# mahfuzalhasan/WaveFormer

Measured on AMD Instinct MI355X. Metric: 128³×4 volumes/sec fwd (1/2/4/8 MI355X) + Dice Δ vs reference, higher is better.
Workload: dtype bf16x3; 1 GPU; MultiscaleTransformer (WaveFormer encoder) forward, 128^3x4 crops; global_batch=8, per_gpu_batch=8, precision=bf16x3, parallelism=replicas x1 (no data-path collective), hip_graph=True

## Files before the change

### waveformer_amd/csrc/ffn.hip

```cpp
#include "kernels.hpp"

namespace wf {

template <typename T>
struct Store4;
template <>
struct Store4<uint16_t> {
  typedef bf16x4 vec;
  static __device__ __forceinline__ f32x4 up(vec u) {
    return f32x4{bf2f((uint16_t)u[0]), bf2f((uint16_t)u[1]), bf2f((uint16_t)u[2]),
                 bf2f((uint16_t)u[3])};
  }
  static __device__ __forceinline__ uint16_t down(float v) { return f2bf(v); }
  static __device__ __forceinline__ vec zero() { return vec{0, 0, 0, 0}; }
  static __device__ __forceinline__ void store4(uint16_t* p, f32x4 v) {
    bf16x4 o;
    o[0] = (short)f2bf(v.x);
    o[1] = (short)f2bf(v.y);
    o[2] = (short)f2bf(v.z);
    o[3] = (short)f2bf(v.w);
    *reinterpret_cast<bf16x4*>(p) = o;
  }
};
template <>
// ... 185 lines not shown
  const int yt = t % nty;
  t /= nty;
  const int zt = t % nzs;
  const int b = t / nzs;
  const int x0 = xt * TX, y0 = yt * TY, z0 = zt * ZS, z1 = min(z0 + ZS, D);
  const int c0 = cc * CH;
  const int tid = threadIdx.x;
  const int cp = tid % (CH / 2), xi = tid / (CH / 2);

  f32x2 w2[27];
#pragma unroll
  for (int k = 0; k < 27; ++k) {
    const int kk = FLIP ? 26 - k : k;
    w2[k] = f32x2{w[(c0 + 2 * cp) * 27 + kk], w[(c0 + 2 * cp + 1) * 27 + kk]};
  }
  const f32x2 bv = bias ? f32x2{bias[c0 + 2 * cp], bias[c0 + 2 * cp + 1]} : f32x2{0.f, 0.f};

  if (LN1) {
    for (int i = tid; i < CH; i += 256) {
      l1w[i] = ln1_w[c0 + i];
      l1b[i] = ln1_b[c0 + i];
    }
    __syncthreads();
  }
  typename V::raw stg[NLD];
  f32x2 st1[LN1 ? NLD : 1];
  bool ok1[LN1 ? NLD : 1];
  const T* src = in + (int64_t)b * D * H * W * Hd + c0;
  auto fetch = [&](int p) {
    const bool pz = p >= 0 && p < D;
    const int pc = min(max(p, 0), D - 1);
#pragma unroll
    for (int j = 0; j < NLD; ++j) {
      const int i = min(j * 256 + tid, PY * PX * NV - 1);
      const int pos = i / NV, v = i - pos * NV;
      const int yy = y0 - 1 + pos / PX, xx = x0 - 1 + pos % PX;
      const bool ok = pz && yy >= 0 && yy < H && xx >= 0 && xx < W;
      const int yc = min(max(yy, 0), H - 1), xc = min(max(xx, 0), W - 1);
      const int64_t gp = ((int64_t)pc * H + yc) * W + xc;
      const typename V::raw u = *reinterpret_cast<const typename V::raw*>(src + gp * Hd + V::N * v);
      stg[j] = ok ? u : V::zero();
      if constexpr (LN1) {
        st1[j] = *reinterpret_cast<const f32x2*>(ln1_stats + ((int64_t)b * D * H * W + gp) * 2);
        ok1[j] = ok;
      }
    }
  };
  auto commit = [&](int buf) {
#pragma unroll
    for (int j = 0; j < NLD; ++j) {
      const int i = j * 256 + tid;
      if (i < PY * PX * NV) {
        if constexpr (LN1) {
          const int v = i % NV;
          const f32x4 lw = *reinterpret_cast<const f32x4*>(l1w + 4 * v);
          const f32x4 lb = *reinterpret_cast<const f32x4*>(l1b + 4 * v);
          const f32x4 y = gelu_erf4((stg[j] - st1[j].x) * st1[j].y * lw + lb);
          stg[j] = ok1[j] ? y : V::zero();
        }
        V::put(pl[buf] + (size_t)i * V::N, stg[j]);
      }
    }
  };

  f32x2 accA[TY], accB[TY], accC[TY];
#pragma unroll
  for (int o = 0; o < TY; ++o) accA[o] = accB[o] = accC[o] = f32x2{0.f, 0.f};
  const int xo = x0 + xi;
  double cs0 = 0.0, cs1 = 0.0, cq0 = 0.0, cq1 = 0.0;
  fetch(z0 - 1);
  commit(0);
  __syncthreads();
  int buf = 0;
  for (int p = z0 - 1; p <= z1; ++p) {
    fetch(p + 1);
    const float* P = pl[buf] + xi * CH + 2 * cp;
#pragma unroll
    for (int r = 0; r < PY; ++r) {
      const f32x2 v0 = *reinterpret_cast<const f32x2*>(P + (r * PX + 0) * CH);
      const f32x2 v1 = *reinterpret_cast<const f32x2*>(P + (r * PX + 1) * CH);
      const f32x2 v2 = *reinterpret_cast<const f32x2*>(P + (r * PX + 2) * CH);
#pragma unroll
      for (int ky = 0; ky < 3; ++ky) {
        const int o = r - ky;
        if (o < 0 || o >= TY) continue;
        const f32x2* w0 = w2 + ky * 3;
        accC[o] = w0[2] * v2 + (w0[1] * v1 + (w0[0] * v0 + accC[o]));
        accB[o] = w0[11] * v2 + (w0[10] * v1 + (w0[9] * v0 + accB[o]));
        accA[o] = w0[20] * v2 + (w0[19] * v1 + (w0[18] * v0 + accA[o]));
      }
    }
    const int zo = p - 1;
    if (zo >= z0) {
      f32x2 r1[TY];
#pragma unroll
      for (int o = 0; o < TY; ++o) r1[o] = Store2<T>::round(accA[o] + bv);
      float mu[TY], m2[TY];
      if (pstats) {
#pragma unroll
        for (int o = 0; o < TY; ++o) mu[o] = group_sum<16>(r1[o].x + r1[o].y) * (1.f / 32.f);
#pragma unroll
        for (int o = 0; o < TY; ++o) {
          const float dx = r1[o].x - mu[o], dy = r1[o].y - mu[o];
          m2[o] = group_sum<16>(dx * dx + dy * dy);
        }
      }
      if (xo < W) {
#pragma unroll
        for (int o = 0; o < TY; ++o) {
          const int yo = y0 + o;
          if (yo < H) {
            const int64_t pos = (((int64_t)b * D + zo) * H + yo) * W + xo;
            Store2<T>::put(out + pos * Hd + c0 + 2 * cp, r1[o]);
            if (cstats) {
              const double a0 = (double)r1[o].x, a1 = (double)r1[o].y;
              cs0 += a0;
              cs1 += a1;
              cq0 += a0 * a0;
              cq1 += a1 * a1;
            }
            if (pstats && cp % (DW_STAT_GROUP / 2) == 0)
              *reinterpret_cast<float2*>(pstats + (pos * (ncc * NG) + cc * NG + cp / (DW_STAT_GROUP / 2)) * 2) =
                  float2{mu[o], m2[o]};
          }
        }
      }
    }
#pragma unroll
    for (int o = 0; o < TY; ++o) {
      accA[o] = accB[o];
      accB[o] = accC[o];
      accC[o] = f32x2{0.f, 0.f};
    }
    commit(buf ^ 1);
    __syncthreads();
    buf ^= 1;
  }
  if (cstats) {
    double* red = reinterpret_cast<double*>(&pl[0][0]);
    double* r = red + (xi * (CH / 2) + cp) * 4;
    r[0] = cs0;
    r[1] = cs1;
    r[2] = cq0;
    r[3] = cq1;
    __syncthreads();
    if (tid < CH * 2) {
      const int pc = tid >> 2, mom = tid & 3;
      double t = 0.0;
#pragma unroll
      for (int xx = 0; xx < TX; ++xx) t += red[(xx * (CH / 2) + pc) * 4 + mom];
      const int c = c0 + 2 * pc + (mom & 1);
      atomicAdd(cstats + ((int64_t)b * Hd + c) * 2 + (mom >> 1), t);
    }
  }
}

int launch_dwconv3d(const void* in, const float* w, const float* b, void* out, float* pstats,
                    int B, int Hd, int D, int H, int W, int prec, hipStream_t s, double* cstats,
                    const float* ln1_stats, const float* ln1_w, const float* ln1_b, int flip) {
  if (Hd % DW_CH != 0) return fail(WF_E_SHAPE, "dwconv3d: hidden width must be a multiple of 32");
  if (flip && (ln1_stats || !store32(prec)))
    return fail(WF_E_SHAPE, "dwconv3d: the mirrored taps are for fp32 data without LN1 staging");
  const bool narrow = W <= 8 && Hd % 64 == 0 && store32(prec) && !flip && !ln1_stats;
  const int dch = narrow ? 64 : DW_CH, dtx = narrow ? 8 : DW_TX;
  const int64_t base = (int64_t)B * (Hd / dch) * cdiv(H, DW_TY) * cdiv(W, dtx);
  int ZS = D;
  const int zmin = narrow ? 4 : 8;
  while (ZS > zmin && base * cdiv(D, ZS) < 2048) ZS = (ZS + 1) / 2;
  const int64_t blocks = base * cdiv(D, ZS);
  if (narrow) {
    hipLaunchKernelGGL((dwconv3d_kernel<float, false, false, 64, 8>), dim3((unsigned)blocks),
                       dim3(256), 0, s, reinterpret_cast<const float*>(in), w, b,
                       reinterpret_cast<float*>(out), pstats, B, Hd, D, H, W, ZS, cstats, nullptr,
                       nullptr, nullptr);
  } else if (ln1_stats) {
    if (!store32(prec) || !ln1_w || !ln1_b)
      return fail(WF_E_SHAPE, "dwconv3d: the LN1 staging needs fp32 h1 and LN1 weights");
    hipLaunchKernelGGL((dwconv3d_kernel<float, true>), dim3((unsigned)blocks), dim3(256), 0, s,
                       reinterpret_cast<const float*>(in), w, b, reinterpret_cast<float*>(out),
                       pstats, B, Hd, D, H, W, ZS, cstats, ln1_stats, ln1_w, ln1_b);
  } else if (store32(prec) && flip)
    hipLaunchKernelGGL((dwconv3d_kernel<float, false, true>), dim3((unsigned)blocks), dim3(256),
                       0, s, reinterpret_cast<const float*>(in), w, b,
                       reinterpret_cast<float*>(out), pstats, B, Hd, D, H, W, ZS, cstats,
                       nullptr, nullptr, nullptr);
  else if (store32(prec))
    hipLaunchKernelGGL((dwconv3d_kernel<float, false>), dim3((unsigned)blocks), dim3(256), 0, s,
                       reinterpret_cast<const float*>(in), w, b, reinterpret_cast<float*>(out),
                       pstats, B, Hd, D, H, W, ZS, cstats, nullptr, nullptr, nullptr);
  else
    hipLaunchKernelGGL((dwconv3d_kernel<uint16_t, false>), dim3((unsigned)blocks), dim3(256), 0,
                       s, reinterpret_cast<const uint16_t*>(in), w, b,
                       reinterpret_cast<uint16_t*>(out), pstats, B, Hd, D, H, W, ZS, cstats,
                       nullptr, nullptr, nullptr);
  return check_launch("dwconv3d");
}

__global__ __launch_bounds__(256) void ln_stats_finalize_kernel(const float* __restrict__ ps,
                                                                int np, int group, float eps,
                                                                float* __restrict__ out,
                                                                int64_t M) {
  const int64_t r = (int64_t)blockIdx.x * 256 + threadIdx.x;
  if (r >= M) return;
  const float2* p = reinterpret_cast<const float2*>(ps) + r * np;
  float mu = 0.f;
  for (int i = 0; i < np; ++i) mu += p[i].x;
  mu *= 1.f / np;
  float m2 = 0.f;
  for (int i = 0; i < np; ++i) {
    const float d = p[i].x - mu;
    m2 += p[i].y + (float)group * d * d;
  }
  *reinterpret_cast<float2*>(out + 2 * r) = float2{mu, rsqrtf(m2 / ((float)np * group) + eps)};
}

int launch_ln_stats_finalize(const float* pstats, int np, int group, float eps, float* out,
                             int64_t M, hipStream_t s) {
  hipLaunchKernelGGL(ln_stats_finalize_kernel, dim3((unsigned)cdiv(M, 256)), dim3(256), 0, s,
                     pstats, np, group, eps, out, M);
  return check_launch("ln_stats_finalize");
}

template <typename T>
static void launch_dw(int tw, dim3 grid, dim3 block, size_t lds, hipStream_t s, const void* in,
                      const float* w, const float* b, const float* ln_w, const float* ln_b,
                      float eps, void* out, int B, int Hd, int D, int H, int W, int R) {
  const T* i = reinterpret_cast<const T*>(in);
  T* o = reinterpret_cast<T*>(out);
  switch (tw) {
    case 2: hipLaunchKernelGGL((dwconv_ln_gelu_kernel<2, T>), grid, block, lds, s, i, w, b, ln_w, ln_b, eps, o, B, Hd, D, H, W, R); break;
    case 4: hipLaunchKernelGGL((dwconv_ln_gelu_kernel<4, T>), grid, block, lds, s, i, w, b, ln_w, ln_b, eps, o, B, Hd, D, H, W, R); break;
    case 8: hipLaunchKernelGGL((dwconv_ln_gelu_kernel<8, T>), grid, block, lds, s, i, w, b, ln_w, ln_b, eps, o, B, Hd, D, H, W, R); break;
    default: hipLaunchKernelGGL((dwconv_ln_gelu_kernel<16, T>), grid, block, lds, s, i, w, b, ln_w, ln_b, eps, o, B, Hd, D, H, W, R); break;
  }
}

int launch_dwconv_ln_gelu(const void* in, const float* w, const float* b, const float* ln_w,
                          const float* ln_b, float eps, void* out, int B, int Hd, int D, int H,
                          int W, int prec, hipStream_t s) {
  if (Hd % 4 != 0) return fail(WF_E_SHAPE, "dwconv: hidden width must be a multiple of 4");
  const int nchunk = Hd / 4;
  if (nchunk > 512) return fail(WF_E_SHAPE, "dwconv: hidden width > 2048 is not supported");
  int R = 256 / nchunk;
  if (R < 1) R = 1;
  if (R > H) R = H;
  int TW = Hd >= 1536 ? 8 : 16;
  while (TW > 2 && (size_t)R * TW * (Hd + 4) * 4 > 64 * 1024) TW >>= 1;
  while (R > 1 && (size_t)R * TW * (Hd + 4) * 4 > 64 * 1024) --R;
  const int threads = (int)cdiv((int64_t)nchunk * R, 64) * 64;
  const int tw_eff = TW > W ? W : TW;
  int tw_t = 16;
  if (tw_eff <= 2) tw_t = 2;
  else if (tw_eff <= 4) tw_t = 4;
  else if (tw_eff <= 8) tw_t = 8;
  const size_t lds = ((size_t)R * tw_t * (Hd + 4) + 2 * (size_t)R * tw_t) * 4;
  const int64_t blocks = (int64_t)B * D * cdiv(H, R) * cdiv(W, tw_t);
  if (store32(prec))
    launch_dw<float>(tw_t, dim3((unsigned)blocks), dim3(threads), lds, s, in, w, b, ln_w, ln_b,
                     eps, out, B, Hd, D, H, W, R);
  else
    launch_dw<uint16_t>(tw_t, dim3((unsigned)blocks), dim3(threads), lds, s, in, w, b, ln_w,
                        ln_b, eps, out, B, Hd, D, H, W, R);
  return check_launch("dwconv_ln_gelu");
}

static DwFcArgs dwfc_args(const void* h1, const float* dw_w, const float* dw_b, const float* ln2_w,
                          const float* ln2_b, float eps2, const uint16_t* fc, const float* fc_b,
                          const float* x, const float* stats, const float* n2_w,
                          const float* n2_b, const float* bscale, float* out, int64_t B, int64_t D,
                          int64_t H, int64_t W) {
  DwFcArgs d{};
  d.h1 = h1;
  d.dw_w = dw_w;
  d.dw_b = dw_b;
  d.ln2_w = ln2_w;
  d.ln2_b = ln2_b;
  d.eps2 = eps2;
  d.fc = fc;
  d.fc_b = fc_b;
  d.x = x;
  d.stats = stats;
  d.n2_w = n2_w;
  d.n2_b = n2_b;
  d.bscale = bscale;
  d.out = out;
  d.B = (int)B;
  d.D = (int)D;
  d.H = (int)H;
  d.W = (int)W;
  return d;
}

}

using namespace wf;

extern "C" int64_t wf_ccf_ffn_workspace_bytes(int64_t B, int64_t C, int64_t hidden, int64_t D,
                                              int64_t H, int64_t W, int precision) {
  const int64_t e = store32(precision) ? 4 : 2;
  const int64_t one = ((B * D * H * W * hidden * e) + 255) & ~(int64_t)255;
  const int64_t st = B * D * H * W * (hidden / DW_STAT_GROUP) * 2 * 4;
  const int64_t s1 = B * D * H * W * 2 * 4;
  const int64_t fcs = C == 192 && hidden == 768 && store32(precision) ? DWFC3_FCS_BYTES : 0;
  return 2 * one + 2 * ((st + 255) & ~(int64_t)255) + ((s1 + 255) & ~(int64_t)255) + fcs;
}

extern "C" int wf_ccf_ffn_stage(int stage, const float* xh, const float* stats,
                                const float* n2_w, const float* n2_b,
                                const uint16_t* pw_bf16x2, const float* pw_b,
                                const float* ln1_w, const float* ln1_b, float eps1,
                                const float* dw_w, const float* dw_b, const float* ln2_w,
                                const float* ln2_b, float eps2, const uint16_t* fc_bf16x2,
                                const float* fc_b, const float* branch_scale, float* out,
                                void* workspace, int64_t B, int64_t C, int64_t hidden,
                                int64_t D, int64_t H, int64_t W, int precision, void* stream) {
  const bool keep = (stage & 16) != 0;
  stage &= ~16;
  WF_REQUIRE(stage >= 0 && stage <= 3, "stage must be 0 (all), 1 (pwconv), 2 (dwconv) or 3 (fc)");
  WF_REQUIRE(B >= 1 && D >= 1 && H >= 1 && W >= 1, "empty volume");
  WF_REQUIRE(C % 8 == 0 && hidden % 8 == 0, "C and hidden must be multiples of 8");
  WF_REQUIRE(valid_prec(precision), "unknown precision");
  WF_REQUIRE_PTR(xh);
  WF_REQUIRE_PTR(pw_bf16x2);
  WF_REQUIRE_PTR(ln1_w);
  WF_REQUIRE_PTR(ln1_b);
  WF_REQUIRE_PTR(dw_w);
  WF_REQUIRE_PTR(dw_b);
  WF_REQUIRE_PTR(ln2_w);
  WF_REQUIRE_PTR(ln2_b);
  WF_REQUIRE_PTR(fc_bf16x2);
  WF_REQUIRE_PTR(out);
  WF_REQUIRE_PTR(workspace);
  if (stats) {
    WF_REQUIRE_PTR(n2_w);
    WF_REQUIRE_PTR(n2_b);
  }
  hipStream_t s = (hipStream_t)stream;
  const int64_t M = B * D * H * W;
  const int64_t e = store32(precision) ? 4 : 2;
  const int64_t one = ((M * hidden * e) + 255) & ~(int64_t)255;
  void* h1 = workspace;
  void* h2 = reinterpret_cast<char*>(workspace) + one;
  const int hbf = !store32(precision);

  GemmArgs g{};
  g.prec = precision;
  g.a_src = xh;
  g.a_bf16 = 0;
  g.a_C = (int)C;
  g.a_nseg = 1;
  g.a_map = MAP_IDENTITY;
  g.a_ln = stats ? LN_GIVEN : LN_NONE;
  g.a_stats = stats;
  g.a_ln_w = n2_w;
  g.a_ln_b = n2_b;
  g.w = pw_bf16x2;
  g.M = M;
  g.N = (int)hidden;
  g.K = (int)C;
  g.epi = EPI_LN_GELU;
  g.bias = pw_b;
  g.e_ln_w = ln1_w;
  g.e_ln_b = ln1_b;
  g.e_eps = eps1;
  g.out = h1;
  g.out_bf16 = hbf;
  g.ldo = hidden;
  int rc = 0;
  const bool split_ln1 = store32(precision) && hidden >= 768 && hidden <= 1536 &&
                         !gemm_lnw_wide_shape(g);
  const bool whole = getenv("WF_FFN_FUSED") != nullptr;
  if (!keep && whole && C == 48 && hidden == 192) {
    if (stage == 1 || stage == 3) return 0;
    DwFcArgs d = dwfc_args(nullptr, dw_w, dw_b, ln2_w, ln2_b, eps2, fc_bf16x2, fc_b, xh, stats, n2_w,
                           n2_b, branch_scale, out, B, D, H, W);
    d.pw = pw_bf16x2;
    d.pw_b = pw_b;
    d.ln1_w = ln1_w;
    d.ln1_b = ln1_b;
    d.eps1 = eps1;
    return launch_ffn_fused(d, precision, s);
  }
  static const bool ln1_pass = getenv("WF_FFN_LN1_FUSE") == nullptr;
  const int64_t stq = ((M * (hidden / DW_STAT_GROUP) * 2 * 4) + 255) & ~(int64_t)255;
  float* pw_pst = reinterpret_cast<float*>(reinterpret_cast<char*>(workspace) + 2 * one + stq);
  float* ln1_st = reinterpret_cast<float*>(reinterpret_cast<char*>(workspace) + 2 * one + 2 * stq);
  int pw_np = 0;
  if (split_ln1 && !keep && !ln1_pass && hidden % DW_STAT_GROUP == 0) {
    GemmArgs g2 = g;
    g2.epi = EPI_STORE;
    const int nt = gemm_kc_pick_nt(g2);
    if (nt > 0 && hidden % (16 * nt) == 0) pw_np = (int)(hidden / (16 * nt));
  }
  if (stage == 0 || stage == 1) {
    if (split_ln1 && pw_np > 0) {
      GemmArgs g2 = g;
      g2.epi = EPI_STORE;
      g2.o_pstats = pw_pst;
      rc = launch_gemm(g2, s, "wf_ccf_ffn_fwd(pwconv)");
      if (!rc)
        rc = launch_ln_stats_finalize(pw_pst, pw_np, (int)(hidden / pw_np), eps1, ln1_st, M, s);
    } else if (split_ln1) {
      GemmArgs g2 = g;
      g2.epi = EPI_STORE;
      rc = launch_gemm(g2, s, "wf_ccf_ffn_fwd(pwconv)");
      if (!rc)
        rc = wf_ln_act_fwd(reinterpret_cast<const float*>(h1), ln1_w, ln1_b, eps1, 1,
                           reinterpret_cast<float*>(h1), M, hidden, stream);
    } else {
      rc = launch_gemm(g, s, "wf_ccf_ffn_fwd(pwconv)");
    }
  }
  if (rc) return rc;
  const bool no_dwfc = getenv("WF_FFN_NO_DWFC") != nullptr;
  const bool dwfc1 = C == 48 && hidden == 192, dwfc2 = C == 96 && hidden == 384;
  const bool dwfc3 = C == 192 && hidden == 768 && store32(precision) && ffn_dwfc3_tb_fits(B, D, H, W);
  if (!keep && !no_dwfc && (dwfc1 || dwfc2 || dwfc3)) {
    if (stage == 1 || stage == 3) return rc;
    DwFcArgs d = dwfc_args(h1, dw_w, dw_b, ln2_w, ln2_b, eps2, fc_bf16x2, fc_b, xh, stats, n2_w,
                           n2_b, branch_scale, out, B, D, H, W);
    if (dwfc3)
      d.fcs = reinterpret_cast<uint16_t*>(
          reinterpret_cast<char*>(workspace) +
          wf_ccf_ffn_workspace_bytes(B, C, hidden, D, H, W, precision) - DWFC3_FCS_BYTES);
    return dwfc1   ? launch_ffn_dwfc_s1(d, precision, s)
           : dwfc2 ? launch_ffn_dwfc2(d, precision, s)
                   : launch_ffn_dwfc3(d, precision, s);
  }
  const bool split_ln = hidden % 32 == 0;
  WF_REQUIRE(!keep || split_ln, "training needs hidden % 32 == 0 (h2 kept pre-LayerNorm)");
  float* pst = reinterpret_cast<float*>(reinterpret_cast<char*>(workspace) + 2 * one);
  if (stage == 0 || stage == 2) {
    if (split_ln && split_ln1 && pw_np > 0)
      rc = launch_dwconv3d(h1, dw_w, dw_b, h2, pst, (int)B, (int)hidden, (int)D, (int)H,
                           (int)W, precision, s, nullptr, ln1_st, ln1_w, ln1_b);
    else if (split_ln)
      rc = launch_dwconv3d(h1, dw_w, dw_b, h2, pst, (int)B, (int)hidden, (int)D, (int)H,
                           (int)W, precision, s);
    else
      rc = launch_dwconv_ln_gelu(h1, dw_w, dw_b, ln2_w, ln2_b, eps2, h2, (int)B, (int)hidden,
                                 (int)D, (int)H, (int)W, precision, s);
  }
  if (rc || stage == 1 || stage == 2) return rc;
  GemmArgs f{};
  f.prec = precision;
  f.a_src = h2;
  f.a_bf16 = hbf;
  f.a_C = (int)hidden;
  f.a_nseg = 1;
  f.a_map = MAP_IDENTITY;
  if (split_ln) {
    f.a_ln = LN_PARTIAL;
    f.a_stats = pst;
    f.a_np = (int)(hidden / DW_STAT_GROUP);
    f.a_ln_w = ln2_w;
    f.a_ln_b = ln2_b;
    f.a_eps = eps2;
    f.a_gelu = 1;
  } else {
    f.a_ln = LN_NONE;
  }
  f.w = fc_bf16x2;
  f.M = M;
  f.N = (int)C;
  f.K = (int)hidden;
  f.epi = EPI_RESID;
  f.bias = fc_b;
  f.r_x = xh;
  f.r_stats = stats;
  f.r_ln_w = n2_w;
  f.r_ln_b = n2_b;
  f.r_scale = branch_scale;
  f.rows_per_sample = D * H * W;
  f.out = out;
  f.out_bf16 = 0;
  f.ldo = C;
  if (!keep) {
    f.kpart = reinterpret_cast<float*>(h1);
    f.kpart_bytes = one;
  }
  return launch_gemm(f, s, "wf_ccf_ffn_fwd(fc)");
}

extern "C" int wf_ccf_ffn_fwd(const float* xh, const float* stats, const float* n2_w,
                              const float* n2_b, const uint16_t* pw_bf16x2, const float* pw_b,
                              const float* ln1_w, const float* ln1_b, float eps1,
                              const float* dw_w, const float* dw_b, const float* ln2_w,
                              const float* ln2_b, float eps2, const uint16_t* fc_bf16x2,
                              const float* fc_b, const float* branch_scale, float* out,
                              void* workspace, int64_t B, int64_t C, int64_t hidden, int64_t D,
                              int64_t H, int64_t W, int precision, void* stream) {
  return wf_ccf_ffn_stage(0, xh, stats, n2_w, n2_b, pw_bf16x2, pw_b, ln1_w, ln1_b, eps1, dw_w,
                          dw_b, ln2_w, ln2_b, eps2, fc_bf16x2, fc_b, branch_scale, out,
                          workspace, B, C, hidden, D, H, W, precision, stream);
}

extern "C" int wf_patch_merging_fwd(const float* x, const float* ln_w, const float* ln_b,
                                    float eps, const uint16_t* red_bf16x2, int v2, float* out,
                                    int64_t B, int64_t C, int64_t D, int64_t H, int64_t W,
                                    int precision, void* stream) {
  WF_REQUIRE(B >= 1 && C % 8 == 0 && C >= 8, "C must be a positive multiple of 8");
  WF_REQUIRE(D % 2 == 0 && H % 2 == 0 && W % 2 == 0 && D >= 2 && H >= 2 && W >= 2,
             "odd sizes (the F.pad branch, wave_helper.py:180-182) are not supported");
  WF_REQUIRE(valid_prec(precision), "unknown precision");
  WF_REQUIRE_PTR(x);
  WF_REQUIRE_PTR(ln_w);
  WF_REQUIRE_PTR(ln_b);
  WF_REQUIRE_PTR(red_bf16x2);
  WF_REQUIRE_PTR(out);
  GemmArgs g{};
  g.prec = precision;
  g.a_src = x;
  g.a_bf16 = 0;
  g.a_C = (int)C;
  g.a_nseg = 8;
  g.a_map = MAP_MERGE;
  g.merge_code = v2 ? 0x76543210 : 0x71251240;
  g.mB = (int)B;
  g.mD = (int)D;
  g.mH = (int)H;
  g.mW = (int)W;
  g.a_ln = LN_COMPUTE;
  g.a_ln_w = ln_w;
  g.a_ln_b = ln_b;
  g.a_eps = eps;
  g.w = red_bf16x2;
  g.M = B * (D / 2) * (H / 2) * (W / 2);
  g.N = (int)(2 * C);
  g.K = (int)(8 * C);
  g.epi = EPI_STORE;
  g.bias = nullptr;
  g.out = out;
  g.out_bf16 = 0;
  g.ldo = 2 * C;
  if (try_launch_merge_resident(g, (hipStream_t)stream)) return check_launch("wf_patch_merging_fwd");
  return launch_gemm(g, (hipStream_t)stream, "wf_patch_merging_fwd");
}
```

### waveformer_amd/csrc/kernels.hpp

```cpp
#pragma once
#include "wf_common.hpp"

namespace wf {

enum Prec { PREC_BF16 = 0, PREC_SPLIT = 1, PREC_FP16 = 2 };

typedef _Float16 f16x4 __attribute__((ext_vector_type(4)));
typedef _Float16 f16x8 __attribute__((ext_vector_type(8)));
__device__ __forceinline__ uint16_t f2h(float f) { return __builtin_bit_cast(uint16_t, (_Float16)f); }

template <int P>
__device__ __forceinline__ uint16_t op_cvt(float x) {
  if constexpr (P == PREC_FP16) return f2h(x);
  else return f2bf(x);
}
template <int P>
__device__ __forceinline__ short op_lo(float x, uint16_t hi) {
  if constexpr (P == PREC_SPLIT) return (short)f2bf(x - bf2f(hi));
  else return (short)0;
}
template <int P>
__device__ __forceinline__ f32x4 mma32(bf16x8 a, bf16x8 b, f32x4 c) {
  if constexpr (P == PREC_FP16)
    return __builtin_amdgcn_mfma_f32_16x16x32_f16(__builtin_bit_cast(f16x8, a),
                                                  __builtin_bit_cast(f16x8, b), c, 0, 0, 0);
  else return __builtin_amdgcn_mfma_f32_16x16x32_bf16(a, b, c, 0, 0, 0);
}
template <int P>
__device__ __forceinline__ f32x4 mma16(bf16x4 a, bf16x4 b, f32x4 c) {
  if constexpr (P == PREC_FP16)
    return __builtin_amdgcn_mfma_f32_16x16x16f16(__builtin_bit_cast(f16x4, a),
                                                 __builtin_bit_cast(f16x4, b), c, 0, 0, 0);
  else return __builtin_amdgcn_mfma_f32_16x16x16bf16_1k(a, b, c, 0, 0, 0);
}
template <int P>
__device__ __forceinline__ f32x4 mma3(f32x4 acc, const bf16x8& w_hi, const bf16x8& w_lo,
                                      const bf16x8& a_hi, const bf16x8& a_lo) {
  if constexpr (P == PREC_SPLIT) {
    acc = mma32<P>(w_hi, a_lo, acc);
    acc = mma32<P>(w_lo, a_hi, acc);
  }
  return mma32<P>(w_hi, a_hi, acc);
}
typedef __bf16 bf16v2 __attribute__((ext_vector_type(2)));
template <int P>
__device__ __forceinline__ void split_pair(float y0, float y1, uint32_t& hi, uint32_t& lo) {
  if constexpr (P == PREC_SPLIT) {
    uint32_t m0, m1;
    asm("s_mov_b32 %0, 0xbf80" : "=s"(m0));
    asm("s_mov_b32 %0, 0xbf800000" : "=s"(m1));
    const bf16v2 h = bf16v2{(__bf16)y0, (__bf16)y1};
    const float r0 = __builtin_amdgcn_fdot2_f32_bf16(h, __builtin_bit_cast(bf16v2, m0), y0, false);
    const float r1 = __builtin_amdgcn_fdot2_f32_bf16(h, __builtin_bit_cast(bf16v2, m1), y1, false);
    hi = __builtin_bit_cast(uint32_t, h);
    lo = __builtin_bit_cast(uint32_t, bf16v2{(__bf16)r0, (__bf16)r1});
  } else {
    hi = (uint32_t)op_cvt<P>(y0) | ((uint32_t)op_cvt<P>(y1) << 16);
    lo = 0;
  }
}
template <int P>
__device__ __forceinline__ void split4(f32x4 v, bf16x4& h, bf16x4& l) {
  uint32_t h0, h1, l0, l1;
  split_pair<P>(v[0], v[1], h0, l0);
  split_pair<P>(v[2], v[3], h1, l1);
  h = __builtin_bit_cast(bf16x4, u32x2{h0, h1});
  l = __builtin_bit_cast(bf16x4, u32x2{l0, l1});
}
template <int P>
__device__ __forceinline__ void split8(const float (&x)[8], bf16x8& h, bf16x8& l) {
  uint32_t hw[4], lw[4];
#pragma unroll
  for (int j = 0; j < 4; ++j) split_pair<P>(x[2 * j], x[2 * j + 1], hw[j], lw[j]);
  h = __builtin_bit_cast(bf16x8, u32x4{hw[0], hw[1], hw[2], hw[3]});
  l = __builtin_bit_cast(bf16x8, u32x4{lw[0], lw[1], lw[2], lw[3]});
}
__host__ __device__ constexpr bool store32(int p) { return p != PREC_BF16; }
inline bool valid_prec(int p) { return p == PREC_BF16 || p == PREC_SPLIT || p == PREC_FP16; }

enum RowMap { MAP_IDENTITY = 0, MAP_WINDOW = 1, MAP_MERGE = 2, MAP_LEVELS = 3 };
constexpr int WF_MAX_LEVELS = 4;
enum LnMode { LN_NONE = 0, LN_GIVEN = 1, LN_COMPUTE = 2, LN_PARTIAL = 3 };
enum EpiMode { EPI_STORE = 0, EPI_LN_GELU = 1, EPI_RESID = 2, EPI_SUBVOXEL = 3 };

struct GemmArgs {
  int prec;
  const void* a_src;
  int a_bf16;
  int a_C;
  int a_nseg;
  int a_map;
  int mB, mD, mH, mW, mws;
  int merge_code;
  int a_ln;
  const float* a_stats;
  int a_np;
  const float* a_ln_w;
  const float* a_ln_b;
  float a_eps;
  int a_gelu;
  const uint16_t* w;
  int64_t M;
  int N, K;
  int epi;
  const float* bias;
  void* out;
  int out_bf16;
  int64_t ldo;
  const float* e_ln_w;
  const float* e_ln_b;
  float e_eps;
  const float* r_x;
  const float* r_stats;
  const float* r_ln_w;
  const float* r_ln_b;
  const float* r_scale;
  int64_t rows_per_sample;
  float* o_pstats;
  float* kpart;
  int64_t kpart_bytes;
  int ksplit;
  const float* lv_src[WF_MAX_LEVELS];
  int lv_row0[WF_MAX_LEVELS];
  int lv_D[WF_MAX_LEVELS], lv_H[WF_MAX_LEVELS], lv_W[WF_MAX_LEVELS];
};

int launch_gemm(const GemmArgs& g, hipStream_t s, const char* who);
int gemm_kc_pick_nt(const GemmArgs& g);
int launch_instnorm_partial(const float* x, int64_t ldx, int64_t B, int64_t C, int64_t P,
                            double* acc, hipStream_t s);
int try_launch_gemm_rows(const GemmArgs& g, hipStream_t s, bool single_chunk_only);

int launch_attn_core(const void* qkv, const float* bias, void* out, float* lse, int64_t Bw,
                     int N, int heads, int hd, float scale, int prec, hipStream_t s,
                     int table_ws = 0, int64_t pair_windows = -1, const GemmArgs* fused = nullptr);
bool attn_tbl_pair_loop(int64_t wh);

int launch_dwconv_ln_gelu(const void* in, const float* w, const float* b, const float* ln_w,
                          const float* ln_b, float eps, void* out, int B, int Hd, int D, int H,
                          int W, int prec, hipStream_t s);
int launch_dwconv3d(const void* in, const float* w, const float* b, void* out, float* pstats,
                    int B, int Hd, int D, int H, int W, int prec, hipStream_t s,
                    double* cstats = nullptr, const float* ln1_stats = nullptr,
                    const float* ln1_w = nullptr, const float* ln1_b = nullptr, int flip = 0);
int launch_ln_stats_finalize(const float* pstats, int np, int group, float eps, float* out,
                             int64_t M, hipStream_t s);
constexpr int DW_STAT_GROUP = 32;
int try_launch_gemm_kc(const GemmArgs& g, hipStream_t s);
int try_launch_merge_resident(const GemmArgs& g, hipStream_t s);
int try_launch_pw2_resident(const GemmArgs& g, hipStream_t s);
int try_launch_gemm_lnw(const GemmArgs& g, hipStream_t s);
bool gemm_lnw_wide_shape(const GemmArgs& g);

}

#include "ffn_dwfc_common.hpp"
```

### waveformer_amd/library.py

```python
from __future__ import annotations

import ctypes
import weakref
from typing import List, Optional, Sequence, Tuple

import torch
from torch import Tensor

from . import _lib, ops
from .autograd import _f32, _p, _s, _scale_rows, colsum, ln_bwd, ln_fwd

DETAIL_KEYS = ops.DETAIL_KEYS
SPLIT = ops.PRECISIONS["bf16x3"]
_FFN_KEEP = 16


def _empty(x: Tensor, dtype=torch.uint8) -> Tensor:
    return x.new_empty((0,), dtype=dtype)


def _round256(n):
    return (n + 255) // 256 * 256


def attn_workspace_bytes(B, C, D1, H1, W1):
    rows = B * D1 * H1 * W1
    return _round256(rows * 3 * C * 4) + _round256(rows * C * 4)


def ffn_workspace_bytes(B, C, hidden, D, H, W):
    M = B * D * H * W
    return (2 * _round256(M * hidden * 4) + 2 * _round256(M * (hidden // 32) * 2 * 4)
            + _round256(M * 2 * 4) + (2 * 192 * 768 * 2 if (C, hidden) == (192, 768) else 0))


@torch.library.custom_op("waveformer::dwt3d", mutates_args=(), device_types="cuda")
def dwt3d(x: Tensor, ln_w: Optional[Tensor], ln_b: Optional[Tensor], eps: float) -> Tensor:
    return ops.dwt3d_haar(x, (ln_w, ln_b, eps) if ln_w is not None else None)


@dwt3d.register_fake
def _(x, ln_w, ln_b, eps):
    B, D, H, W, C = x.shape
    return x.new_empty((8, B, D // 2, H // 2, W // 2, C))


def _dwt3d_setup(ctx, inputs, output):
    x, ln_w, ln_b, eps = inputs
    ctx.save_for_backward(x, ln_w, ln_b)
    ctx.eps = eps


@torch.library.custom_op("waveformer::dwt3d_backward", mutates_args=(), device_types="cuda")
def dwt3d_backward(gbands: Tensor, x: Tensor, ln_w: Optional[Tensor], ln_b: Optional[Tensor],
                   eps: float) -> Tuple[Tensor, Tensor, Tensor]:
    B, D, H, W, C = x.shape
    g = gbands.contiguous()
    ptrs = [g[k].data_ptr() for k in range(8)]
    strides = []
    for k in range(8):
        strides.extend(g[k].stride())
    dx = torch.empty_like(x)
    _lib.call("wf_dwt3d_haar_bwd", (ctypes.c_void_p * 8)(*ptrs), (ctypes.c_int64 * 40)(*strides),
              dx.data_ptr(), B, C, D, H, W, _s())
    if ln_w is None:
        return dx, _empty(x, torch.float32), _empty(x, torch.float32)
    dx2, dw, db = ln_bwd(x.view(-1, C), ln_w, ln_b, eps, False, dx.view(-1, C))
    return dx2.view(B, D, H, W, C), dw, db


@dwt3d_backward.register_fake
def _(gbands, x, ln_w, ln_b, eps):
    if ln_w is None:
        return torch.empty_like(x), _empty(x, torch.float32), _empty(x, torch.float32)
    return torch.empty_like(x), torch.empty_like(ln_w), torch.empty_like(ln_b)


def _dwt3d_bwd(ctx, gbands):
    x, ln_w, ln_b = ctx.saved_tensors
    dx, dw, db = torch.ops.waveformer.dwt3d_backward(gbands, x, ln_w, ln_b, ctx.eps)
    return dx, (dw if ln_w is not None else None), (db if ln_w is not None else None), None


dwt3d.register_autograd(_dwt3d_bwd, setup_context=_dwt3d_setup)


@torch.library.custom_op("waveformer::idwt3d", mutates_args=(), device_types="cuda")
def idwt3d(ll: Tensor, details: List[Tensor]) -> Tensor:
    L = len(details) // 7
    dets = [dict(zip(DETAIL_KEYS, details[7 * l:7 * l + 7])) for l in range(L)]
    return ops.idwt3d_haar(ll, dets)


@idwt3d.register_fake
def _(ll, details):
    L = len(details) // 7
    B, C, d, h, w = ll.shape
    s = 2 ** L
    return ll.new_empty((B, C, d * s, h * s, w * s))


def _idwt3d_setup(ctx, inputs, output):
    ll, details = inputs
    ctx.L = len(details) // 7
    ctx.save_for_backward(ll)


@torch.library.custom_op("waveformer::idwt3d_backward", mutates_args=(), device_types="cuda")
def idwt3d_backward(gout: Tensor, ll: Tensor, levels: int) -> List[Tensor]:
    B, C, d, h, w = ll.shape
    L = levels
    cur = _f32(gout)
    per_level: List[List[Tensor]] = [None] * L
    for l in range(L - 1, -1, -1):
        s = 2 ** l
        dl, hl, wl = d * s, h * s, w * s
        lo = torch.empty((B, C, dl, hl, wl), dtype=torch.float32, device=cur.device)
        dets = [torch.empty((B, dl, hl, wl, C), dtype=torch.float32,
                            device=cur.device).permute(0, 4, 1, 2, 3) for _ in range(7)]
        parr = (ctypes.c_void_p * 7)(*[t.data_ptr() for t in dets])
        sarr = (ctypes.c_int64 * 5)(*dets[0].stride())
        _lib.call("wf_haar_analysis_ncdhw", cur.data_ptr(), cur.stride(0), cur.stride(1),
                  lo.data_ptr(), parr, sarr, B, C, dl, hl, wl, _s())
        per_level[l] = dets
        cur = lo
    return [cur] + [t for lv in per_level for t in lv]


@idwt3d_backward.register_fake
def _(gout, ll, levels):
    B, C, d, h, w = ll.shape
    out = [ll.new_empty((B, C, d, h, w))]
    for l in range(levels):
        s = 2 ** l
        out += [ll.new_empty((B, d * s, h * s, w * s, C)).permute(0, 4, 1, 2, 3)
                for _ in range(7)]
    return out


def _idwt3d_bwd(ctx, gout):
    (ll,) = ctx.saved_tensors
    g = torch.ops.waveformer.idwt3d_backward(gout, ll, ctx.L)
    return g[0], list(g[1:])


idwt3d.register_autograd(_idwt3d_bwd, setup_context=_idwt3d_setup)


@torch.library.custom_op("waveformer::wavedec3_level", mutates_args=(), device_types="cuda")
def wavedec3_level(x: Tensor, wavelet: str) -> Tensor:
    return ops.dwt3d(x, wavelet)


@wavedec3_level.register_fake
def _(x, wavelet):
    L = ops.wavelet_taps(wavelet)
    B, C, D, H, W = x.shape
    return x.new_empty((8, B, C, (D + L - 1) // 2, (H + L - 1) // 2, (W + L - 1) // 2))


def _wavedec3_setup(ctx, inputs, output):
    x, wavelet = inputs
    ctx.size = tuple(x.shape[2:])
    ctx.wavelet = wavelet


@torch.library.custom_op("waveformer::wavedec3_level_backward", mutates_args=(),
                         device_types="cuda")
def wavedec3_level_backward(gbands: Tensor, size: List[int], wavelet: str) -> Tensor:
    return ops.dwt3d_bwd(gbands, size, wavelet)


@wavedec3_level_backward.register_fake
def _(gbands, size, wavelet):
    return gbands.new_empty((gbands.shape[1], gbands.shape[2]) + tuple(size))


def _wavedec3_bwd(ctx, gbands):
    return torch.ops.waveformer.wavedec3_level_backward(gbands, list(ctx.size),
                                                        ctx.wavelet), None


wavedec3_level.register_autograd(_wavedec3_bwd, setup_context=_wavedec3_setup)


@torch.library.custom_op("waveformer::waverec3_level", mutates_args=(), device_types="cuda")
def waverec3_level(ll: Tensor, details: List[Tensor], wavelet: str) -> Tensor:
    if len(details) != 7:
        raise ValueError(f"waverec3_level: expected 7 details, got {len(details)}")
    return ops.waverec3([ll, dict(zip(DETAIL_KEYS, details))], wavelet)


@waverec3_level.register_fake
def _(ll, details, wavelet):
    L = ops.wavelet_taps(wavelet)
    B, C, nz, ny, nx = details[0].shape
    return ll.new_empty((B, C, 2 * nz - L + 2, 2 * ny - L + 2, 2 * nx - L + 2))


def _is_cl(t: Tensor) -> bool:
    return t.shape[1] > 1 and t.stride(1) == 1 and not t.is_contiguous()


def _waverec3_setup(ctx, inputs, output):
    ll, details, wavelet = inputs
    ctx.ll_size = tuple(ll.shape[2:])
    ctx.cl = [_is_cl(t) for t in [ll] + list(details)]
    ctx.wavelet = wavelet


@torch.library.custom_op("waveformer::waverec3_level_backward", mutates_args=(),
                         device_types="cuda")
def waverec3_level_backward(gout: Tensor, ll_size: List[int], channel_last: List[bool],
                            wavelet: str) -> List[Tensor]:
    return ops.idwt3d_level_bwd(gout, ll_size, wavelet, channel_last)


@waverec3_level_backward.register_fake
def _(gout, ll_size, channel_last, wavelet):
    L = ops.wavelet_taps(wavelet)
    B, C = gout.shape[:2]
    n = tuple((o + L - 2) // 2 for o in gout.shape[2:])
    out = []
    for k in range(8):
        shp = tuple(ll_size) if k == 0 else n
        out.append(gout.new_empty((B,) + shp + (C,)).permute(0, 4, 1, 2, 3) if channel_last[k]
                   else gout.new_empty((B, C) + shp))
    return out


def _waverec3_bwd(ctx, gout):
    g = torch.ops.waveformer.waverec3_level_backward(gout, list(ctx.ll_size), ctx.cl,
                                                     ctx.wavelet)
    return g[0], list(g[1:]), None


waverec3_level.register_autograd(_waverec3_bwd, setup_context=_waverec3_setup)


@torch.library.custom_op("waveformer::window_attn", mutates_args=(), device_types="cuda")
def window_attn(x: Tensor, ln_w: Optional[Tensor], ln_b: Optional[Tensor], eps: float,
                wqkv: Tensor, bqkv: Optional[Tensor], table: Tensor, index: Tensor,
                wproj: Tensor, bproj: Optional[Tensor], ws: int, heads: int, scale: float,
                prec: int, train: bool, index_formula: bool = False
                ) -> Tuple[Tensor, Tensor, Tensor]:
    C = x.shape[-1]
    ln = (ln_w, ln_b, eps) if ln_w is not None else None
    if not train:
        bias = ops.attention_bias(table, index, ws, heads, C // heads, index_formula)
        out = ops.window_attention(x, wqkv, bqkv, bias, wproj, bproj, ws, heads, scale, ln,
                                   prec=prec)
        return out, _empty(x), _empty(x, torch.float32)
    B, D1, H1, W1, _ = x.shape
    N = ws ** 3
    bias = ops.rel_pos_bias(table.detach(), index)
    wq, wp = ops.split_weight(wqkv, prec=SPLIT), ops.split_weight(wproj, prec=SPLIT)
    out = torch.empty_like(x)
    wsb = _lib.query("wf_window_attention_workspace_bytes", B, C, D1, H1, W1, SPLIT)
    work = torch.empty(wsb, dtype=torch.uint8, device=x.device)
    lse = torch.empty(B * D1 * H1 * W1 * heads, dtype=torch.float32, device=x.device)
    _lib.call("wf_window_attention_fwd_train", x.data_ptr(), _p(ln_w), _p(ln_b), float(eps),
              wq.data_ptr(), _p(bqkv), bias.data_ptr(), wp.data_ptr(), _p(bproj),
              out.data_ptr(), work.data_ptr(), lse.data_ptr(), B, C, D1, H1, W1, ws, heads,
              float(scale), SPLIT, _s())
    return out, work, lse


@window_attn.register_fake
def _(x, ln_w, ln_b, eps, wqkv, bqkv, table, index, wproj, bproj, ws, heads, scale, prec,
      train, index_formula=False):
    if not train:
        return torch.empty_like(x), _empty(x), _empty(x, torch.float32)
    B, D1, H1, W1, C = x.shape
    wsb = attn_workspace_bytes(B, C, D1, H1, W1)
    return (torch.empty_like(x), x.new_empty((wsb,), dtype=torch.uint8),
            x.new_empty((B * D1 * H1 * W1 * heads,), dtype=torch.float32))


def _attn_setup(ctx, inputs, output):
    (x, ln_w, ln_b, eps, wqkv, bqkv, table, index, wproj, bproj, ws, heads, scale, prec,
     train, _formula) = inputs
    _, work, lse = output
    ctx.meta = (ws, heads, float(scale), float(eps), bool(train))
    ctx.save_for_backward(x, ln_w, ln_b, wqkv, bqkv, table, index, wproj, bproj, work, lse)
    ctx.set_materialize_grads(False)


def _wgrad(dy: Tensor, x: Tensor) -> Tensor:
    return ops.gemm_tn(dy, x)


_INDEX_GROUPS: dict = {}


def _index_groups(index: Tensor, rows: int) -> Tuple[Tensor, Tensor]:
    key = (index.data_ptr(), index._version, tuple(index.shape), rows, str(index.device))
    hit = _INDEX_GROUPS.get(key)
    if hit is not None and hit[0]() is index:
        return hit[1], hit[2]
    flat = index.reshape(-1)
    vals, perm = torch.sort(flat, stable=True)
    offsets = torch.searchsorted(vals, torch.arange(rows + 1, device=index.device,
                                                    dtype=vals.dtype))
    perm, offsets = perm.contiguous(), offsets.to(torch.int64).contiguous()
    if len(_INDEX_GROUPS) >= 64:
        _INDEX_GROUPS.clear()
    _INDEX_GROUPS[key] = (weakref.ref(index), perm, offsets)
    return perm, offsets


@torch.library.custom_op("waveformer::window_attn_backward", mutates_args=(),
                         device_types="cuda")
def window_attn_backward(gout: Tensor, x: Tensor, ln_w: Optional[Tensor],
                         ln_b: Optional[Tensor], wqkv: Tensor, bqkv: Optional[Tensor],
                         table: Tensor, index: Tensor, wproj: Tensor, bproj: Optional[Tensor],
                         work: Tensor, lse: Tensor, eps: float, ws: int, heads: int,
                         scale: float) -> Tuple[Tensor, Tensor, Tensor, Tensor, Tensor, Tensor,
                                                Tensor, Tensor]:
    if work.numel() == 0:
        raise RuntimeError("waveformer::window_attn: backward of a train=False call")
    B, D1, H1, W1, C = x.shape
    N = ws ** 3
    rows = B * D1 * H1 * W1
    E = lambda: _empty(x, torch.float32)
    bias = ops.rel_pos_bias(table.detach(), index)
    qkv_bytes = _round256(rows * 3 * C * 4)
    qkv = work[:rows * 3 * C * 4].view(torch.float32).view(rows, 3 * C)
    o = work[qkv_bytes:qkv_bytes + rows * C * 4].view(torch.float32).view(rows, C)
    g = _f32(gout).view(rows, C)
    dwproj = _wgrad(g, o)
    dbproj = colsum(g) if bproj is not None else E()
    do = ops.mm_rows(g, wproj)
    dqkv = torch.empty((rows, 3 * C), dtype=torch.float32, device=x.device)
    dbias = torch.empty((heads, N, N), dtype=torch.float32, device=x.device)
    bws = torch.empty(_lib.query("wf_window_attention_bwd_workspace_bytes", B, C, D1, H1, W1, ws,
                                 heads), dtype=torch.uint8, device=x.device)
# ... 388 lines not shown
```

Measured before the change: 1306 volumes/s.

## Add register-streamed 16-row GEMM kernels for stage-4 FFN pwconv and fc

Adds a specialized GEMM path for the C=384, hidden=1536 FFN where each workgroup handles 16 rows and every wave streams its own slice of a pre-permuted weight buffer through registers with triple buffering. A small kernel first reorders the pwconv and fc weights (both split planes) into a wave-contiguous stream in workspace. The pwconv GEMM now fuses the LN+GELU epilogue with an in-block row reduction, and the fc GEMM uses dedicated loader waves to apply the partial-stat LayerNorm to A while the compute waves run. This replaces the generic gemm plus stats-finalize launches and the k-partitioned fc, at the cost of a weight reshuffle on every call and more workspace.

```diff
diff --git a/waveformer_amd/csrc/ffn.hip b/waveformer_amd/csrc/ffn.hip
--- a/waveformer_amd/csrc/ffn.hip
+++ b/waveformer_amd/csrc/ffn.hip
@@ -511,7 +511,8 @@
   const int64_t st = B * D * H * W * (hidden / DW_STAT_GROUP) * 2 * 4;
   const int64_t s1 = B * D * H * W * 2 * 4;
   const int64_t fcs = C == 192 && hidden == 768 && store32(precision) ? DWFC3_FCS_BYTES : 0;
-  return 2 * one + 2 * ((st + 255) & ~(int64_t)255) + ((s1 + 255) & ~(int64_t)255) + fcs;
+  const int64_t r16s = C == 384 && hidden == 1536 && store32(precision) ? 2 * R16_W_BYTES : 0;
+  return 2 * one + 2 * ((st + 255) & ~(int64_t)255) + ((s1 + 255) & ~(int64_t)255) + fcs + r16s;
 }
 
 extern "C" int wf_ccf_ffn_stage(int stage, const float* xh, const float* stats,
@@ -594,15 +595,21 @@
   const int64_t stq = ((M * (hidden / DW_STAT_GROUP) * 2 * 4) + 255) & ~(int64_t)255;
   float* pw_pst = reinterpret_cast<float*>(reinterpret_cast<char*>(workspace) + 2 * one + stq);
   float* ln1_st = reinterpret_cast<float*>(reinterpret_cast<char*>(workspace) + 2 * one + 2 * stq);
+  const bool r16 = !keep && C == 384 && hidden == 1536 && store32(precision) && M <= R16_MAX_ROWS;
+  uint16_t* r16_ws = reinterpret_cast<uint16_t*>(
+      reinterpret_cast<char*>(workspace) +
+      wf_ccf_ffn_workspace_bytes(B, C, hidden, D, H, W, precision) - 2 * R16_W_BYTES);
   int pw_np = 0;
-  if (split_ln1 && !keep && !ln1_pass && hidden % DW_STAT_GROUP == 0) {
+  if (split_ln1 && !keep && !ln1_pass && !r16 && hidden % DW_STAT_GROUP == 0) {
     GemmArgs g2 = g;
     g2.epi = EPI_STORE;
     const int nt = gemm_kc_pick_nt(g2);
     if (nt > 0 && hidden % (16 * nt) == 0) pw_np = (int)(hidden / (16 * nt));
   }
   if (stage == 0 || stage == 1) {
-    if (split_ln1 && pw_np > 0) {
+    if (r16) {
+      rc = launch_gemm_r16(g, 0, fc_bf16x2, r16_ws, s);
+    } else if (split_ln1 && pw_np > 0) {
       GemmArgs g2 = g;
       g2.epi = EPI_STORE;
       g2.o_pstats = pw_pst;
@@ -684,6 +691,7 @@
   f.out = out;
   f.out_bf16 = 0;
   f.ldo = C;
+  if (r16 && split_ln) return launch_gemm_r16(f, 1, nullptr, r16_ws, s);
   if (!keep) {
     f.kpart = reinterpret_cast<float*>(h1);
     f.kpart_bytes = one;
diff --git a/waveformer_amd/csrc/gemm_r16.hip b/waveformer_amd/csrc/gemm_r16.hip
--- /dev/null
+++ b/waveformer_amd/csrc/gemm_r16.hip
@@ -0,0 +1,309 @@
+#include "gemm_common.hpp"
+
+namespace wf {
+
+#ifndef WF_R16_DBG
+#define WF_R16_DBG 0
+#endif
+
+namespace r16 {
+constexpr int C = 384, HID = 1536;
+constexpr int NTW = 3;
+constexpr int NR = 3;
+template <int SITE>
+struct Geo;
+template <>
+struct Geo<0> {
+  static constexpr int K = C, N = HID, NWV = 16, NPASS = 2, NLW = 0, KSEG = 2 * (C / 32);
+};
+template <>
+struct Geo<1> {
+  static constexpr int K = HID, N = C, NWV = 8, NPASS = 1, NLW = 8, KSEG = 16;
+};
+static_assert(Geo<0>::NWV * Geo<0>::NPASS * NTW * 16 == Geo<0>::N, "pwconv columns");
+static_assert(Geo<1>::NWV * Geo<1>::NPASS * NTW * 16 == Geo<1>::N, "fc columns");
+static_assert((int64_t)2 * C * HID * 2 == R16_W_BYTES, "one weight, two planes");
+static_assert(Geo<1>::KSEG * 32 == 64 * 8 && Geo<1>::NLW * 2 == 16, "fc loader: a wave-load per row and third");
+}
+
+template <int NPL, int SITE>
+__device__ __forceinline__ void r16_stream_one(const uint16_t* __restrict__ w,
+                                               uint16_t* __restrict__ out, int i) {
+  typedef r16::Geo<SITE> G;
+  constexpr int KS = G::K / 32;
+  const int lane = i & 63;
+  int r = i >> 6;
+  const int pl = r % NPL;
+  r /= NPL;
+  const int t = r % r16::NTW;
+  r /= r16::NTW;
+  const int ks = r % KS;
+  r /= KS;
+  const int n = (r * r16::NTW + t) * 16 + (lane & 15), k = ks * 32 + 8 * (lane >> 4);
+  *reinterpret_cast<bf16x8*>(out + (size_t)i * 8) =
+      *reinterpret_cast<const bf16x8*>(w + (size_t)pl * G::N * G::K + (size_t)n * G::K + k);
+}
+template <int NPL>
+__global__ __launch_bounds__(256) void r16_stream_kernel(const uint16_t* __restrict__ pw,
+                                                          const uint16_t* __restrict__ fc,
+                                                          uint16_t* __restrict__ out) {
+  constexpr int NF = r16::C * r16::HID / 8 * NPL;
+  static_assert(NF % 256 == 0, "whole workgroups per weight");
+  const int i = blockIdx.x * 256 + threadIdx.x;
+  if (i < NF) r16_stream_one<NPL, 0>(pw, out, i);
+  else if (i < 2 * NF) r16_stream_one<NPL, 1>(fc, out + R16_W_BYTES / 2, i - NF);
+}
+
+template <int P, int SITE, bool INPLACE = false>
+__global__ __launch_bounds__((r16::Geo<SITE>::NWV + r16::Geo<SITE>::NLW) * 64, 1) void gemm_r16_kernel(
+    GemmArgs g, const uint16_t* __restrict__ wstream, int dbg_) {
+  typedef r16::Geo<SITE> G;
+  using r16::NR;
+  using r16::NTW;
+  constexpr bool SPLIT = P == PREC_SPLIT;
+  constexpr int NPL = SPLIT ? 2 : 1;
+  constexpr int K = G::K, N = G::N, NWV = G::NWV, NLW = G::NLW, NPASS = G::NPASS, KSEG = G::KSEG;
+  constexpr int KS = K / 32, NS = NPASS * KS;
+  constexpr int NT = NPASS * NTW;
+  constexpr int AS = K + WF_LDS_KPAD;
+  __shared__ __attribute__((aligned(16))) uint16_t As[NPL * 16 * AS];
+  __shared__ float red[NLW ? 1 : NWV][16];
+  __shared__ __attribute__((aligned(16))) float lnv[NLW ? 2 * K : 4];
+  const int dbg = WF_R16_DBG ? dbg_ : 0;
+  const int64_t M = g.M;
+  const int tid = threadIdx.x, lane = tid & 63, wid = tid >> 6;
+  const int l15 = lane & 15, g4 = lane >> 4;
+  const int64_t r0 = (int64_t)blockIdx.x * 16;
+  const int64_t orow = r0 + l15, orowc = min(orow, M - 1);
+  auto bar = [&]() {
+    asm volatile("s_waitcnt lgkmcnt(0)" ::: "memory");
+    __builtin_amdgcn_s_barrier();
+    asm volatile("" ::: "memory");
+  };
+
+  if constexpr (NLW > 0) {
+    if (wid >= NWV) {
+      constexpr int NSEG = KS / KSEG, SEGC = KSEG * 32;
+      const int lw = wid - NWV, ltid = tid - NWV * 64;
+      float v[NSEG][2][8];
+      if (!(dbg & 1)) {
+#pragma unroll
+        for (int q = 0; q < NSEG; ++q)
+#pragma unroll
+          for (int j = 0; j < 2; ++j)
+            load8f<false>(g.a_src, min(r0 + lw + 8 * j, M - 1) * K + q * SEGC + 8 * lane, v[q][j]);
+      }
+      float pmean = 0.f, prstd = 1.f;
+      ln_partial_combine(g.a_stats + orowc * g.a_np * 2, g.a_np, K, g.a_eps, g4, pmean, prstd);
+      float mean[2], rstd[2];
+#pragma unroll
+      for (int j = 0; j < 2; ++j) {
+        mean[j] = __shfl(pmean, lw + 8 * j, 64);
+        rstd[j] = __shfl(prstd, lw + 8 * j, 64);
+      }
+      for (int i = ltid; i < 2 * K / 4; i += NLW * 64)
+        reinterpret_cast<f32x4*>(lnv)[i] =
+            i < K / 4 ? reinterpret_cast<const f32x4*>(g.a_ln_w)[i]
+                      : reinterpret_cast<const f32x4*>(g.a_ln_b)[i - K / 4];
+      bar();
+#pragma unroll
+      for (int q = 0; q < NSEG; ++q) {
+        if (!(dbg & 1)) {
+#pragma unroll
+          for (int j = 0; j < 2; ++j) {
+            const int k = q * SEGC + 8 * lane;
+            bf16x8 ah, al;
+            a_fragment<P>(v[q][j], mean[j], rstd[j], lnv, lnv + K, k, true, true, g.a_gelu != 0, ah, al);
+            *reinterpret_cast<bf16x8*>(As + (lw + 8 * j) * AS + k) = ah;
+            if (SPLIT) *reinterpret_cast<bf16x8*>(As + 16 * AS + (lw + 8 * j) * AS + k) = al;
+          }
+        }
+        bar();
+      }
+      return;
+    }
+    __builtin_amdgcn_s_setprio(3);
+  }
+
+  const __amdgpu_buffer_rsrc_t wrsrc = buf_rsrc(wstream, NPL * N * K * 2);
+  const int wvoff = wid * (NS * NTW * NPL * 1024) + 16 * lane;
+  const bf16x8 z8 = {0, 0, 0, 0, 0, 0, 0, 0};
+  bf16x8 wh[NR][NTW], wl[NR][NTW];
+  auto wload = [&](int s) {
+    const int sl = s % NR;
+#pragma unroll
+    for (int t = 0; t < NTW; ++t) {
+      if constexpr (INPLACE) {
+        const uint16_t* p = g.w + (size_t)(((wid * NPASS + s / KS) * NTW + t) * 16 + l15) * K +
+                            (s % KS) * 32 + 8 * g4;
+        wh[sl][t] = *reinterpret_cast<const bf16x8*>(p);
+        wl[sl][t] = SPLIT ? *reinterpret_cast<const bf16x8*>(p + (size_t)N * K) : z8;
+        continue;
+      }
+      const int so = (s * NTW + t) * NPL * 1024;
+      wh[sl][t] = __builtin_bit_cast(bf16x8, __builtin_amdgcn_raw_buffer_load_b128(wrsrc, wvoff, so, 0));
+      wl[sl][t] = SPLIT ? __builtin_bit_cast(bf16x8, __builtin_amdgcn_raw_buffer_load_b128(
+                                                         wrsrc, wvoff, so + 1024, 0))
+                        : z8;
+    }
+  };
+  wload(0);
+  wload(1);
+
+  const int cw = wid * (NT * 16);
+  f32x4 xr[SITE == 1 ? NT : 1];
+  float rm_ = 0.f, rs_ = 1.f, bs = 1.f;
+  if constexpr (SITE == 1) {
+#pragma unroll
+    for (int t = 0; t < NT; ++t)
+      xr[t] = *reinterpret_cast<const f32x4*>(g.r_x + orowc * N + cw + 16 * t + 4 * g4);
+    if (g.r_stats) {
+      rm_ = g.r_stats[2 * orowc];
+      rs_ = g.r_stats[2 * orowc + 1];
+    }
+    if (g.r_scale) bs = g.r_scale[orowc / g.rows_per_sample];
+  }
+
+  if constexpr (NLW == 0) {
+    if (!(dbg & 1)) {
+      constexpr int NTH = NWV * 64, OPR = K / 8, NIT = (16 * OPR + NTH - 1) / NTH;
+      float v[NIT][8], mean[NIT], rstd[NIT];
+#pragma unroll
+      for (int j = 0; j < NIT; ++j) {
+        const int i = min(tid + NTH * j, 16 * OPR - 1);
+        const int r = i / OPR, o = i - r * OPR;
+        const int64_t row = min(r0 + r, M - 1);
+        load8f<false>(g.a_src, row * K + 8 * o, v[j]);
+        mean[j] = 0.f;
+        rstd[j] = 1.f;
+        if (g.a_ln == LN_GIVEN) {
+          mean[j] = g.a_stats[2 * row];
+          rstd[j] = g.a_stats[2 * row + 1];
+        }
+      }
+#pragma unroll
+      for (int j = 0; j < NIT; ++j) {
+        const int i = tid + NTH * j;
+        const int ic = min(i, 16 * OPR - 1);
+        const int r = ic / OPR, o = ic - r * OPR;
+        bf16x8 ah, al;
+        a_fragment<P>(v[j], mean[j], rstd[j], g.a_ln_w, g.a_ln_b, 8 * o, true, g.a_ln != LN_NONE,
+                      g.a_gelu != 0, ah, al);
+        if (i < 16 * OPR) {
+          *reinterpret_cast<bf16x8*>(As + r * AS + 8 * o) = ah;
+          if (SPLIT) *reinterpret_cast<bf16x8*>(As + 16 * AS + r * AS + 8 * o) = al;
+        }
+      }
+    }
+    __syncthreads();
+  } else {
+    bar();
+    bar();
+  }
+
+  f32x4 acc[NT];
+#pragma unroll
+  for (int t = 0; t < NT; ++t) acc[t] = f32x4{0.f, 0.f, 0.f, 0.f};
+  auto lds8 = [](const uint16_t* q) { return *reinterpret_cast<const bf16x8*>(q); };
+  const uint16_t* Ap = As + l15 * AS + 8 * g4;
+  bf16x8 ah = lds8(Ap), al = SPLIT ? lds8(Ap + 16 * AS) : z8;
+#pragma unroll
+  for (int s = 0; s < NS; ++s) {
+    if (s + 2 < NS) wload(s + 2);
+    __builtin_amdgcn_sched_barrier(0);
+#pragma unroll
+    for (int t = 0; t < NTW; ++t)
+      acc[(s / KS) * NTW + t] = mma3<P>(acc[(s / KS) * NTW + t], wh[s % NR][t], wl[s % NR][t], ah, al);
+    __builtin_amdgcn_sched_barrier(0);
+    if (s + 1 < NS) {
+      if (NLW > 0 && (s + 1) % KSEG == 0) bar();
+      const int k1 = ((s + 1) % KS) * 32;
+      ah = lds8(Ap + k1);
+      al = SPLIT ? lds8(Ap + 16 * AS + k1) : z8;
+    }
+  }
+
+  if (dbg & 2) {
+    const float s = tile_sum<NT>(acc);
+    if (s == 1.2345f) reinterpret_cast<float*>(g.out)[tid] = s;
+    return;
+  }
+
+#pragma unroll
+  for (int t = 0; t < NT; ++t)
+    if (g.bias) acc[t] += *reinterpret_cast<const f32x4*>(g.bias + cw + 16 * t + 4 * g4);
+  if constexpr (SITE == 0) {
+    auto wsum = [&](int r) {
+      float t = (red[0][r] + red[1][r]) + (red[2][r] + red[3][r]);
+#pragma unroll
+      for (int w = 4; w < NWV; w += 4) t += (red[w][r] + red[w + 1][r]) + (red[w + 2][r] + red[w + 3][r]);
+      return t;
+    };
+    const float s = tile_sum<NT>(acc);
+    if (g4 == 0) red[wid][l15] = s;
+    __syncthreads();
+    const float mean = wsum(l15) * (1.f / N);
+    __syncthreads();
+    const float q = tile_sqdev<NT>(acc, mean);
+    if (g4 == 0) red[wid][l15] = q;
+    __syncthreads();
+    const float rstd = rsqrtf(wsum(l15) * (1.f / N) + g.e_eps);
+#pragma unroll
+    for (int t = 0; t < NT; ++t) {
+      const int col = cw + 16 * t + 4 * g4;
+      const f32x4 lw = *reinterpret_cast<const f32x4*>(g.e_ln_w + col) * 0.5f;
+      const f32x4 lb = *reinterpret_cast<const f32x4*>(g.e_ln_b + col) * 0.5f;
+      const f32x4 v = gelu_half4((acc[t] - mean) * rstd * lw + lb);
+      if (orow < M) store4(g.out, false, orow * g.ldo, col, v);
+    }
+  } else {
+#pragma unroll
+    for (int t = 0; t < NT; ++t) {
+      const int col = cw + 16 * t + 4 * g4;
+      const f32x4 v = resid_epilogue(acc[t], xr[t], rm_, rs_, g.r_ln_w + col, g.r_ln_b + col, bs,
+                                     g.r_stats != nullptr);
+      if (orow < M) store4(g.out, false, orow * g.ldo, col, v);
+    }
+  }
+}
+
+int launch_gemm_r16(const GemmArgs& g, int site, const uint16_t* fc_w, uint16_t* wstream,
+                    hipStream_t s) {
+  using namespace r16;
+  const bool shape = site == 0 ? (g.K == C && g.N == HID && g.epi == EPI_LN_GELU && fc_w &&
+                                  (g.a_ln == LN_NONE || g.a_ln == LN_GIVEN) && !g.a_gelu)
+                               : (g.K == HID && g.N == C && g.epi == EPI_RESID &&
+                                  g.a_ln == LN_PARTIAL && g.a_np > 0 && HID % g.a_np == 0);
+  if (!shape || g.a_map != MAP_IDENTITY || g.a_bf16 || g.out_bf16 || g.a_C != g.K ||
+      !(g.prec == PREC_SPLIT || g.prec == PREC_FP16) || g.M < 1 || g.M > R16_MAX_ROWS ||
+      g.ldo < g.N || g.ldo % 4 != 0)
+    return fail(WF_E_SHAPE, "gemm_r16: not the stage-4 CCF_FFN pwconv / fc");
+  if (!wstream) return fail(WF_E_SHAPE, "gemm_r16: no workspace for the streamed weights");
+  const int dbg = WF_R16_DBG && getenv("WF_R16_DBG") ? atoi(getenv("WF_R16_DBG")) : 0;
+  const bool split = g.prec == PREC_SPLIT;
+  const dim3 grid((unsigned)cdiv(g.M, 16));
+  const uint16_t* ws = wstream + (site == 0 ? 0 : R16_W_BYTES / 2);
+  if (site == 0 && !(dbg & 4)) {
+    const int nblk = 2 * (C * HID / 8 * (split ? 2 : 1) / 256);
+    if (split) hipLaunchKernelGGL(r16_stream_kernel<2>, dim3(nblk), dim3(256), 0, s, g.w, fc_w, wstream);
+    else hipLaunchKernelGGL(r16_stream_kernel<1>, dim3(nblk), dim3(256), 0, s, g.w, fc_w, wstream);
+  }
+  auto go = [&](auto gemm_k, int nw) {
+    hipLaunchKernelGGL(gemm_k, grid, dim3(nw * 64), 0, s, g, ws, dbg);
+  };
+  constexpr int NW0 = Geo<0>::NWV + Geo<0>::NLW, NW1 = Geo<1>::NWV + Geo<1>::NLW;
+#if WF_R16_DBG
+  if ((dbg & 4) && split) {
+    if (site == 0) go(gemm_r16_kernel<PREC_SPLIT, 0, true>, NW0);
+    else go(gemm_r16_kernel<PREC_SPLIT, 1, true>, NW1);
+    return check_launch("gemm_r16");
+  }
+#endif
+  if (site == 0 && split) go(gemm_r16_kernel<PREC_SPLIT, 0>, NW0);
+  else if (site == 0) go(gemm_r16_kernel<PREC_FP16, 0>, NW0);
+  else if (split) go(gemm_r16_kernel<PREC_SPLIT, 1>, NW1);
+  else go(gemm_r16_kernel<PREC_FP16, 1>, NW1);
+  return check_launch("gemm_r16");
+}
+
+}
diff --git a/waveformer_amd/csrc/kernels.hpp b/waveformer_amd/csrc/kernels.hpp
--- a/waveformer_amd/csrc/kernels.hpp
+++ b/waveformer_amd/csrc/kernels.hpp
@@ -151,6 +151,10 @@
 int try_launch_pw2_resident(const GemmArgs& g, hipStream_t s);
 int try_launch_gemm_lnw(const GemmArgs& g, hipStream_t s);
 bool gemm_lnw_wide_shape(const GemmArgs& g);
+constexpr int64_t R16_W_BYTES = 2 * 384 * 1536 * 2;
+constexpr int64_t R16_MAX_ROWS = (int64_t)1 << 30;
+int launch_gemm_r16(const GemmArgs& g, int site, const uint16_t* fc_w, uint16_t* wstream,
+                    hipStream_t s);
 
 }
 
diff --git a/waveformer_amd/library.py b/waveformer_amd/library.py
--- a/waveformer_amd/library.py
+++ b/waveformer_amd/library.py
@@ -31,7 +31,8 @@
 def ffn_workspace_bytes(B, C, hidden, D, H, W):
     M = B * D * H * W
     return (2 * _round256(M * hidden * 4) + 2 * _round256(M * (hidden // 32) * 2 * 4)
-            + _round256(M * 2 * 4) + (2 * 192 * 768 * 2 if (C, hidden) == (192, 768) else 0))
+            + _round256(M * 2 * 4) + (2 * 192 * 768 * 2 if (C, hidden) == (192, 768) else 0)
+            + (2 * 2 * 384 * 1536 * 2 if (C, hidden) == (384, 1536) else 0))
 
 
 @torch.library.custom_op("waveformer::dwt3d", mutates_args=(), device_types="cuda")
```

Result: no change. 1319 volumes/s, median of 6 (+1.0%).
